# IamJasonBian/Splendor-RL-Gym

Measured on NVIDIA B200. Metric: expanded states/sec (gen+dedup+score+top-k), higher is better.
Workload: dtype u64 keys / f64 scores

## Files before the change

### splendor-rl-gym_b200/csrc/spl_kernels.cuh

```cuda
#pragma once
#include "spl_common.cuh"

namespace spl {

struct Counters {
    unsigned long long total_cands;
    unsigned long long n_new;
    unsigned long long n_emitted;
    unsigned long long sk_min, sk_max;
    long long goal_rank;
    unsigned int error;
    unsigned int ticket[4];
    unsigned long long key_or[2], key_and[2];
    unsigned long long n_buys;
    unsigned int n_runs, n_new_nodes;
    unsigned int n_cls[8];
    unsigned long long n_ties;
};

struct SelState {
    unsigned long long prefix;
    unsigned long long k_rem;
    unsigned long long c_gt;
    unsigned long long tie_count;
// ... 2 lines not shown
};

struct SmemTabs {
    uint64_t buy_lo[NCOL][8];
    uint64_t buy_hi[NCOL][8];
    uint32_t card[SPL_NUM_CARDS + 2];
};

__device__ __forceinline__ void load_tabs(SmemTabs &s, const DevTables *__restrict__ g) {
    const uint64_t *src = reinterpret_cast<const uint64_t *>(g);
    uint64_t *dst = reinterpret_cast<uint64_t *>(&s);
    for (int i = threadIdx.x; i < 2 * NCOL * 8; i += blockDim.x) dst[i] = src[i];
    for (int i = threadIdx.x; i < SPL_NUM_CARDS; i += blockDim.x) s.card[i] = g->card[i];
}

__device__ __forceinline__ void derive_parent(const SmemTabs &s, const uint32_t *__restrict__ takes_idx, uint64_t lo,
                                              uint64_t hi, uint64_t aux, uint64_t &bm_lo, uint64_t &bm_hi,
                                              uint32_t &nb, uint32_t &tk) {
    const uint32_t g = (uint32_t)(lo & GEM_MASK);
    bm_lo = ~lo;
    bm_hi = ~hi & HI_KEY_MASK;
#pragma unroll
    for (int c = 0; c < NCOL; ++c) {
        uint32_t v = ((g >> (3 * c)) & 7) + (uint32_t)((aux >> (24 + 5 * c)) & 31);
        v = v > 7 ? 7 : v;
        bm_lo &= s.buy_lo[c][v];
        bm_hi &= s.buy_hi[c][v];
    }
    nb = __popcll(bm_lo) + __popcll(bm_hi);
    tk = __ldg(takes_idx + g);
}

__device__ __forceinline__ int nth_set_bit64(uint64_t m, int n) {
    const uint32_t l = (uint32_t)m, h = (uint32_t)(m >> 32);
    const int c = __popc(l);
    return n < c ? nth_set_bit32(l, n) : 32 + nth_set_bit32(h, n - c);
}

__device__ __forceinline__ void make_child(const SmemTabs &s, const uint16_t *__restrict__ takes_edges, uint64_t lo,
                                           uint64_t hi, uint64_t aux, uint64_t bm_lo, uint64_t bm_hi, uint32_t nb,
                                           uint32_t tk, uint32_t ord, uint64_t &clo, uint64_t &chi, uint64_t &caux) {
    if (ord < nb) {
        const int c0 = __popcll(bm_lo);
        const int pos = (int)ord < c0 ? nth_set_bit64(bm_lo, ord) : 64 + nth_set_bit64(bm_hi, ord - c0);
        const uint32_t cd = s.card[pos - 15];
// ... 188 lines not shown
    cd = s.card[pos - 15];
    const uint32_t g = (uint32_t)(lo & GEM_MASK);
    uint32_t ng = 0;
    saved = 0;
#pragma unroll
    for (int c = 0; c < NCOL; ++c) {
        const int cost = (cd >> (3 * c)) & 7;
        const int b = (int)((aux >> (24 + 5 * c)) & 31);
        const int gc = (g >> (3 * c)) & 7;
        const int pay = max(cost - b, 0);
        saved += cost - pay;
        ng |= (uint32_t)max(gc - pay, 0) << (3 * c);
    }
    return ng;
}

constexpr int BUY_WIN = 4096;

struct ExpandSmem2 {
    SmemTabs tabs;
    uint64_t lo[TILE], hi[TILE], aux[TILE];
    uint32_t tk[TILE], nb[TILE], pref[TILE], prefb[TILE + 1];
    uint16_t units[TILE / 32][128];
    uint16_t blist[BUY_WIN];
    uint32_t warp_sums[TILE / 32 + 1];
};

template <int MODE, int IDENT>
__global__ void __launch_bounds__(TILE) expand_kernel(const Rec *__restrict__ front, int64_t n_par,
                                                      const DevTables *__restrict__ tabs,
// ... 58 lines not shown
                ++q;
            }
            m = bm_hi;
            while (m) {
                const int pos = 64 + __ffsll((long long)m) - 1;
                m &= m - 1;
                if (q >= w0 && q < w0 + BUY_WIN) S.blist[q - w0] = (uint16_t)(tid << 7 | pos);
                ++q;
            }
        }
        __syncthreads();
        const uint32_t nbw = min((uint32_t)BUY_WIN, total_buys - w0);
        for (uint32_t i = tid; i < nbw; i += TILE) {
            const uint32_t ent = S.blist[i], j = ent >> 7;
            const int pos = ent & 127;
            const uint64_t lo = S.lo[j], aux = S.aux[j];
            uint32_t saved, cd;
            const uint32_t ng = buy_gems(S.tabs, lo, aux, pos, saved, cd);
            uint64_t klo = (lo & ~GEM_MASK) | ng, khi = S.hi[j];
            if (pos < 64) klo |= 1ull << pos; else khi |= 1ull << (pos - 64);
            const uint32_t ord = w0 + i - S.prefb[j];
            const uint32_t tt = c0 + S.pref[j] + ord;
            if (MODE == MODE_PROBE) {
                cand_slot[tt] = probe_ident<IDENT>(table, cap, tag, klo, khi, ~(uint64_t)tt, n_new, &ctr->error);
            } else {
                const uint64_t caux = aux + saved + ((uint64_t)((cd >> 15) & 7) << 16) + (1ull << (24 + 5 * ((cd >> 18) & 7)));
                Rec r{klo, khi, caux, ((uint64_t)(rank_base + p0 + j) << 8) | ord};
                st_rec(cand_out + tt, r);
            }
        }
    }
    if (MODE == MODE_PROBE) {
#pragma unroll
        for (int d = 16; d; d >>= 1) n_new += __shfl_xor_sync(0xffffffffu, n_new, d);
        if (lane == 0 && n_new) atomicAdd(&ctr->n_new, (unsigned long long)n_new);
    }
}

template <int IDENT>
__global__ void __launch_bounds__(TILE) probe_list_kernel(const spl_key *__restrict__ keys, int64_t n,
                                                          uint64_t *__restrict__ table, uint64_t cap, uint64_t tag,
// ... 1025 lines not shown
```

### splendor-rl-gym_b200/csrc/spl_m2.cuh

```cuda
#pragma once
#include "spl_kernels.cuh"

namespace spl {

constexpr int GEM_STATES = 2898;
constexpr int NODE_BM_WORDS = 46;
constexpr int NODE_WORDS = 48;
constexpr uint64_t NODE_OCC = 1ull << 63;
constexpr int SMALL_ITEMS = 32;
constexpr int SMALL_W = 128;
constexpr int SM_TBL = 256;
constexpr int SM_STAGE = 48;
struct GroupArgs;
constexpr int NUM_CLS = 8;
constexpr int CLS_WARP = 6, CLS_CTA = 7;
constexpr int M2_WARPS = TILE / 32;
constexpr int BIG_DONE = 16;
constexpr int BIG_AT_BITS = 24;

__device__ __host__ __forceinline__ void mask_words(uint64_t lo, uint64_t hi, uint64_t &m0, uint64_t &m1) {
    m0 = (lo >> 15) | (hi << 49);
    m1 = (hi & HI_KEY_MASK) >> 15;
}
__device__ __host__ __forceinline__ uint64_t mask_hash(uint64_t m0, uint64_t m1) { return hash_key(m0, m1); }

__device__ __forceinline__ uint64_t node_find_or_create(uint64_t *__restrict__ nodes, uint64_t nn, uint64_t m0, uint64_t m1,
                                                        bool &fresh, unsigned int *error) {
    const uint64_t want1 = m1 | NODE_OCC;
    uint64_t i = __umul64hi(mask_hash(m0, m1), nn);
    fresh = false;
    for (int probes = 0; probes < MAX_PROBE; ++probes) {
        uint64_t *N = nodes + i * NODE_WORDS;
        uint64_t a, b;
// ... 74 lines not shown
    const uint32_t excl = block_excl_scan(nb, warp_sums, total);
    if (threadIdx.x < 32) {
        const uint64_t e = lookback_exclusive(status, tile, total, 0);
        if (threadIdx.x == 0) {
            s_base = e;
            if (total_tk) atomicAdd(&ctr->total_cands, (unsigned long long)total_tk);
            if ((int64_t)(tile + 1) * TILE >= np) ctr->n_buys = e + total;
        }
    }
    __syncthreads();
    if (p < np) boff[p] = (uint32_t)(s_base + excl);
}

struct BuySmem {
    SmemTabs tabs;
    uint64_t lo[TILE], hi[TILE], aux[TILE];
    uint32_t prefb[TILE + 1];
    uint16_t blist[BUY_WIN];
    uint32_t warp_sums[TILE / 32 + 1];
};
__global__ void __launch_bounds__(TILE) m2_buys_kernel(const Rec *__restrict__ front, int64_t np,
                                                       const DevTables *__restrict__ tabs,
                                                       const uint32_t *__restrict__ takes_idx,
                                                       const uint32_t *__restrict__ boff, int64_t rank_base,
                                                       Rec *__restrict__ brec, uint64_t *__restrict__ iv) {
    extern __shared__ __align__(16) unsigned char smem_raw[];
    BuySmem &S = *reinterpret_cast<BuySmem *>(smem_raw);
    const unsigned tid = threadIdx.x;
    load_tabs(S.tabs, tabs);
    __syncthreads();
    const int64_t p0 = (int64_t)blockIdx.x * TILE, p = p0 + tid;
    const uint32_t b0 = boff[p0];
    uint64_t bm_lo = 0, bm_hi = 0;
    uint32_t nb = 0, tk = 0;
    if (p < np) {
        Rec r;
        ld_rec(front + p, r);
        derive_parent(S.tabs, takes_idx, r.lo, r.hi, r.aux, bm_lo, bm_hi, nb, tk);
        S.lo[tid] = r.lo; S.hi[tid] = r.hi; S.aux[tid] = r.aux;
    }
    uint32_t total_buys;
    const uint32_t prefb = block_excl_scan(nb, S.warp_sums, total_buys);
    S.prefb[tid] = prefb;
    if (tid == 0) S.prefb[TILE] = total_buys;
    for (uint32_t w0 = 0; w0 < total_buys; w0 += BUY_WIN) {
        __syncthreads();
        {
            uint32_t q = prefb;
            uint64_t m = bm_lo;
            while (m) {
                const int pos = __ffsll((long long)m) - 1;
                m &= m - 1;
                if (q >= w0 && q < w0 + BUY_WIN) S.blist[q - w0] = (uint16_t)(tid << 7 | pos);
                ++q;
            }
            m = bm_hi;
            while (m) {
                const int pos = 64 + __ffsll((long long)m) - 1;
                m &= m - 1;
                if (q >= w0 && q < w0 + BUY_WIN) S.blist[q - w0] = (uint16_t)(tid << 7 | pos);
                ++q;
            }
        }
        __syncthreads();
        const uint32_t nbw = min((uint32_t)BUY_WIN, total_buys - w0);
        for (uint32_t i = tid; i < nbw; i += TILE) {
            const uint32_t ent = S.blist[i], j = ent >> 7;
            const int pos = ent & 127;
            const uint64_t lo = S.lo[j], aux = S.aux[j];
            uint32_t saved, cd;
            const uint32_t ng = buy_gems(S.tabs, lo, aux, pos, saved, cd);
            uint64_t klo = (lo & ~GEM_MASK) | ng, khi = S.hi[j];
            if (pos < 64) klo |= 1ull << pos; else khi |= 1ull << (pos - 64);
            const uint32_t ord = w0 + i - S.prefb[j];
            const uint64_t caux = aux + saved + ((uint64_t)((cd >> 15) & 7) << 16) + (1ull << (24 + 5 * ((cd >> 18) & 7)));
            const uint64_t g = (uint64_t)b0 + w0 + i;
            Rec r{klo, khi, caux, ((uint64_t)(rank_base + p0 + j) << 8) | ord};
            st_rec(brec + g, r);
            uint64_t m0, m1;
            mask_words(klo, khi, m0, m1);
            iv[np + g] = (mask_hash(m0, m1) & 0xFFFFFFFF00000000ull) | (uint64_t)(np + g);
        }
    }
}

__global__ void __launch_bounds__(TILE, 4) psort_scatter_kernel(const uint64_t *__restrict__ v_in, int64_t n, int shift,
                                                                const uint32_t *__restrict__ matrix_scanned, uint32_t ntiles,
                                                                uint64_t *__restrict__ v_out) {
    __shared__ uint32_t whist[TILE / 32][SORT_BINS];
    __shared__ uint32_t dbase[SORT_BINS], gbase[SORT_BINS];
    __shared__ uint32_t warp_sums[TILE / 32 + 1];
    __shared__ uint64_t stage[SORT_TILE];
    const unsigned lane = threadIdx.x & 31, w = threadIdx.x >> 5;
    for (int i = threadIdx.x; i < (TILE / 32) * SORT_BINS; i += TILE) (&whist[0][0])[i] = 0;
    __syncthreads();
    const int64_t tbase = (int64_t)blockIdx.x * SORT_TILE, wbase = tbase + (int64_t)w * (32 * SORT_ITEMS);
// ... 285 lines not shown
    uint64_t *nodes;
    uint64_t nn;
    Rec *out;
    uint64_t *out_sk;
    uint64_t out_base;
    uint32_t *cls_list[NUM_CLS];
    int h, noise_mode;
    ScoreLuts L;
    Counters *ctr;
};

__device__ __forceinline__ uint32_t item_id(const GroupArgs &A, uint32_t i) { return (uint32_t)A.iv[i]; }
__device__ __forceinline__ uint64_t parent_rank(const GroupArgs &A, uint32_t id) {
    return A.grank ? A.grank[id] : (uint64_t)(A.rank_base + id);
}

constexpr int M2_WARPS_ = TILE / 32;
struct WarpStage {
    uint64_t *st;
    uint32_t cnt;
    uint64_t kmin, kmax;
    __device__ __forceinline__ uint64_t &lo(uint32_t i) const { return st[i]; }
    __device__ __forceinline__ uint64_t &hi(uint32_t i) const { return st[1 * M2_WARPS_ * SM_STAGE + i]; }
    __device__ __forceinline__ uint64_t &aux(uint32_t i) const { return st[2 * M2_WARPS_ * SM_STAGE + i]; }
    __device__ __forceinline__ uint64_t &link(uint32_t i) const { return st[3 * M2_WARPS_ * SM_STAGE + i]; }
    __device__ __forceinline__ uint64_t &sk(uint32_t i) const { return st[4 * M2_WARPS_ * SM_STAGE + i]; }
};
__device__ __forceinline__ void stage_flush(const GroupArgs &A, WarpStage &W) {
    const unsigned lane = threadIdx.x & 31;
    __syncwarp();
// ... 93 lines not shown
    const bool act = q < (ptk & 0xff);
    const uint32_t g = act ? (uint32_t)__ldg(A.takes_edges + (ptk >> 8) + q) : 0u;
    bm_step(A, W, bm, act, true, g, (pgr << 8) | (pnb + q), (plo & ~GEM_MASK) | g, phi, paux);
}
__device__ __forceinline__ void take_steps(const GroupArgs &A, WarpStage &W, uint64_t *bm, uint64_t plo, uint64_t phi, uint64_t paux,
                                           uint64_t pgr, uint32_t ptk, uint32_t pnb) {
    const unsigned lane = threadIdx.x & 31;
    const uint32_t ntk = ptk & 0xff;
    for (uint32_t q0 = 0; q0 < ntk; q0 += 32) {
        const uint32_t q = q0 + lane;
        const bool act = q < ntk;
        const uint32_t g = act ? (uint32_t)__ldg(A.takes_edges + (ptk >> 8) + q) : 0u;
        bm_step(A, W, bm, act, false, g, (pgr << 8) | (pnb + q), (plo & ~GEM_MASK) | g, phi, paux);
    }
}
__device__ __forceinline__ void load_item(const GroupArgs &A, const SmemTabs &tabs, uint32_t i, Rec &it, bool &isP, uint32_t &nb,
                                          uint32_t &tk, uint64_t &grank, uint64_t &m0, uint64_t &m1) {
    const uint32_t id = item_id(A, i);
    isP = id < A.np;
    nb = tk = 0;
    grank = 0;
    if (isP) {
        ld_rec(A.front + id, it);
        uint64_t bl, bh;
        derive_parent(tabs, A.takes_idx, it.lo, it.hi, it.aux, bl, bh, nb, tk);
        grank = parent_rank(A, id);
    } else {
        ld_rec(A.brec + (id - A.np), it);
        grank = it.link >> 8;
    }
    mask_words(it.lo, it.hi, m0, m1);
}
__device__ __forceinline__ void warp_epilogue(const GroupArgs &A, WarpStage &W, uint32_t n_fresh) {
    const unsigned lane = threadIdx.x & 31;
    if (W.cnt) stage_flush(A, W);
    if (lane == 0 && n_fresh) atomicAdd(&A.ctr->n_new_nodes, n_fresh);
    if (A.out_sk) {
#pragma unroll
        for (int d = 16; d; d >>= 1) {
            W.kmin = min(W.kmin, __shfl_xor_sync(0xffffffffu, W.kmin, d));
            W.kmax = max(W.kmax, __shfl_xor_sync(0xffffffffu, W.kmax, d));
        }
        if (lane == 0 && W.kmin <= W.kmax) {
            atomicMin(&A.ctr->sk_min, (unsigned long long)W.kmin);
            atomicMax(&A.ctr->sk_max, (unsigned long long)W.kmax);
// ... 65 lines not shown
                        if (x > i) {
                            const uint64_t a = bs[i], b = bs[x];
                            if ((a > b) == ((i & k) == 0)) { bs[i] = b; bs[x] = a; }
                        }
                    }
                    __syncwarp();
                }
        }
        uint64_t (*done)[2] = S.done[w];
        int n_done = 0;
        uint32_t lead = s;
        while (lead != 0xFFFFFFFFu) {
            uint64_t M0 = 0, M1 = 0;
            if (lane == 0) {
                const uint32_t id = item_id(A, lead);
                const Rec *src = id < A.np ? A.front + id : A.brec + (id - A.np);
                mask_words(src->lo, src->hi, M0, M1);
            }
            M0 = __shfl_sync(0xffffffffu, M0, 0); M1 = __shfl_sync(0xffffffffu, M1, 0);
            uint64_t *N = node_open(A, M0, M1, bm, n_fresh);
            uint32_t next_lead = 0xFFFFFFFFu;
            Rec it{0, 0, 0, 0}, bt{0, 0, 0, 0};
            uint32_t nb = 0, tk = 0;
            uint64_t grank = 0, brank = 0;
            uint32_t bnext = pe, pnext = s;
            unsigned bmask = 0, pmask = 0;
            for (;;) {
                if (!pmask && pnext < pe) {
                    const bool valid = pnext + lane < pe;
                    bool p_;
                    uint64_t m0 = 0, m1 = 0;
                    if (valid) load_item(A, S.tabs, pnext + lane, it, p_, nb, tk, grank, m0, m1);
                    const bool ok = valid && m0 == M0 && m1 == M1;
                    bool other = valid && !ok;
#pragma unroll
                    for (int d = 0; d < MAX_SETS; ++d) other = other && !(d < n_done && done[d][0] == m0 && done[d][1] == m1);
                    const unsigned om = __ballot_sync(0xffffffffu, other);
                    if (om) next_lead = min(next_lead, pnext + (uint32_t)__ffs(om) - 1);
                    pmask = __ballot_sync(0xffffffffu, ok);
                    pnext += 32;
                    continue;
                }
                if (!bmask && bnext < e) {
                    const bool valid = bnext + lane < e;
                    uint64_t m0 = 0, m1 = 0;
                    if (valid) {
                        const uint32_t at = resort ? pe + (uint32_t)(bs[bnext - pe + lane] & 1023u) : bnext + lane;
                        ld_rec(A.brec + (item_id(A, at) - A.np), bt);
                        mask_words(bt.lo, bt.hi, m0, m1);
                        brank = bt.link >> 8;
                    }
                    const bool ok = valid && m0 == M0 && m1 == M1;
                    bool other = valid && !ok;
#pragma unroll
                    for (int d = 0; d < MAX_SETS; ++d) other = other && !(d < n_done && done[d][0] == m0 && done[d][1] == m1);
                    const unsigned om = __ballot_sync(0xffffffffu, other);
                    if (om) {
                        const uint32_t j = bnext - pe + (uint32_t)__ffs(om) - 1;
                        next_lead = min(next_lead, resort ? pe + (uint32_t)(bs[j] & 1023u) : pe + j);
                    }
                    bmask = __ballot_sync(0xffffffffu, ok);
                    bnext += 32;
                    continue;
// ... 35 lines not shown
        }
      }
    }
    warp_epilogue(A, W, n_fresh);
}

constexpr int TINY_ITEMS = 16;
#ifndef SPL_BIG_W
#define SPL_BIG_W 1024
#endif
constexpr uint32_t BIG_W = SPL_BIG_W;
template <bool UNORDERED>
__global__ void __launch_bounds__(TILE) m2_group_tiny_kernel(GroupArgs A, uint32_t n_runs) {
    __shared__ uint32_t warp_sums[TILE / 32 + 1];
    __shared__ uint64_t s_base;
    const unsigned lane = threadIdx.x & 31;
    const uint32_t r = blockIdx.x * TILE + threadIdx.x;
    int cls = -1;
    uint32_t s = 0, cnt = 0, winmask = 0;
    uint64_t *N = nullptr;
    uint32_t n_fresh = 0;
    uint64_t kmin = ~0ull, kmax = 0;
    if (r < n_runs) {
        s = A.run_start[r];
        cnt = A.run_start[r + 1] - s;
        const uint32_t id0 = item_id(A, s);
        const uint32_t wgt = A.run_wpre[r + 1] - A.run_wpre[r];
        if (cnt <= TINY_ITEMS && id0 >= A.np) cls = 0;
        else cls = wgt <= A.warp_max ? CLS_WARP : CLS_CTA;
        if (cls == 0) {
            uint64_t lo0, hi0, M0, M1;
            ld_cg_u64x2(reinterpret_cast<const uint64_t *>(A.brec + (id0 - A.np)), lo0, hi0);
            mask_words(lo0, hi0, M0, M1);
            uint32_t gp[TINY_ITEMS / 2];
#pragma unroll
            for (int q = 0; q < TINY_ITEMS / 2; ++q) gp[q] = 0;
            gp[0] = (uint32_t)(lo0 & GEM_MASK);
            bool same = true;
#pragma unroll
            for (int j = 1; j < TINY_ITEMS; ++j) {
                if (j < (int)cnt) {
                    uint64_t lo, hi, m0, m1;
                    ld_cg_u64x2(reinterpret_cast<const uint64_t *>(A.brec + (item_id(A, s + j) - A.np)), lo, hi);
                    mask_words(lo, hi, m0, m1);
                    same = same && m0 == M0 && m1 == M1;
                    gp[j >> 1] |= (uint32_t)(lo & GEM_MASK) << (16 * (j & 1));
                }
            }
            if (!same) {
                cls = CLS_WARP;
            } else {
                bool fresh;
                const uint64_t node = node_find_or_create(A.nodes, A.nn, M0, M1, fresh, &A.ctr->error);
                n_fresh = fresh;
                N = A.nodes + node * NODE_WORDS;
#pragma unroll
                for (int j = 0; j < TINY_ITEMS; ++j) {
                    if (j < (int)cnt) {
// ... 22 lines not shown
        if (m) {
            uint32_t base = 0;
            if (lane == (unsigned)(__ffs(m) - 1)) base = atomicAdd(&A.ctr->n_cls[k], (unsigned)__popc(m));
            base = __shfl_sync(0xffffffffu, base, __ffs(m) - 1);
            if (cls == k) A.cls_list[k][base + __popc(m & ((1u << lane) - 1))] = r;
        }
    }
    uint32_t tot;
    const uint32_t ex = block_excl_scan(__popc(winmask), warp_sums, tot);
    if (threadIdx.x == 0 && tot) s_base = A.out_base + atomicAdd(&A.ctr->n_emitted, (unsigned long long)tot);
    __syncthreads();
    uint64_t pos = s_base + ex;
    for (uint32_t m = winmask; m; m &= m - 1) {
        const int j = __ffs(m) - 1;
        Rec it;
        ld_rec(A.brec + (item_id(A, s + j) - A.np), it);
        st_rec(A.out + pos, it);
        const uint64_t k = flip_f64((uint64_t)__double_as_longlong(score_state(A.h, A.noise_mode, it.lo, it.hi & HI_KEY_MASK, it.aux, A.L)));
        A.out_sk[pos] = k;
        kmin = min(kmin, k); kmax = max(kmax, k);
        const uint32_t rk = __ldg(A.gemrank + (uint32_t)(it.lo & GEM_MASK));
        atomicOr(reinterpret_cast<unsigned long long *>(N + 2 + (rk >> 6)), 1ull << (rk & 63));
        ++pos;
    }
#pragma unroll
    for (int d = 16; d; d >>= 1) {
        n_fresh += __shfl_xor_sync(0xffffffffu, n_fresh, d);
        kmin = min(kmin, __shfl_xor_sync(0xffffffffu, kmin, d));
        kmax = max(kmax, __shfl_xor_sync(0xffffffffu, kmax, d));
    }
    if (lane == 0 && n_fresh) atomicAdd(&A.ctr->n_new_nodes, n_fresh);
// ... 1 lines not shown
        atomicMin(&A.ctr->sk_min, (unsigned long long)kmin);
        atomicMax(&A.ctr->sk_max, (unsigned long long)kmax);
    }
}

struct BigSmem {
    SmemTabs tabs;
    uint64_t tbl[GEM_STATES + 6];
    uint64_t bm[NODE_BM_WORDS];
    uint64_t done0[BIG_DONE], done1[BIG_DONE];
    uint32_t warp_sums[TILE / 32 + 1];
    uint32_t job, next, fresh, n_done;
    uint64_t node, base, m0, m1;
};

template <class F>
__device__ __forceinline__ void big_enumerate(const GroupArgs &A, BigSmem &S, uint32_t s, uint32_t e, uint64_t M0, uint64_t M1, F &&f) {
    for (uint32_t i = s + threadIdx.x; i < e; i += TILE) {
        const uint32_t id = item_id(A, i);
        Rec it;
        const bool isP = id < A.np;
        if (isP) ld_rec(A.front + id, it); else ld_rec(A.brec + (id - A.np), it);
        uint64_t m0, m1;
        mask_words(it.lo, it.hi, m0, m1);
        if (m0 != M0 || m1 != M1) {
            bool done = false;
            for (uint32_t d = 0; d < S.n_done; ++d) done |= (S.done0[d] == m0 && S.done1[d] == m1);
            if (!done) atomicMin(&S.next, i);
            continue;
        }
        if (!isP) {
            f((uint32_t)__ldg(A.gemrank + (uint32_t)(it.lo & GEM_MASK)), it.link, i - s);
        } else {
            uint64_t bl, bh;
            uint32_t nb, tk;
            derive_parent(S.tabs, A.takes_idx, it.lo, it.hi, it.aux, bl, bh, nb, tk);
            const uint64_t tb = (parent_rank(A, id) << 8) | nb;
            const uint32_t ntk = tk & 0xff;
            for (uint32_t q = 0; q < ntk; ++q) f((uint32_t)__ldg(A.gemrank + __ldg(A.takes_edges + (tk >> 8) + q)), tb + q, i - s);
        }
    }
}

__global__ void __launch_bounds__(TILE) m2_group_big_kernel(GroupArgs A) {
    extern __shared__ __align__(16) unsigned char smem_raw[];
    BigSmem &S = *reinterpret_cast<BigSmem *>(smem_raw);
    const unsigned tid = threadIdx.x, lane = tid & 31;
    load_tabs(S.tabs, A.tabs);
    const uint32_t n_big = A.ctr->n_cls[CLS_CTA];
    uint32_t n_fresh = 0;
    uint64_t kmin = ~0ull, kmax = 0;
    uint32_t ticket = 0;
    if (tid == 0) ticket = atomicAdd(&A.ctr->ticket[3], 1u);
    for (;;) {
        __syncthreads();
        if (tid == 0) {
            S.job = ticket;
            if (ticket < n_big) ticket = atomicAdd(&A.ctr->ticket[3], 1u);
        }
        __syncthreads();
        if (S.job >= n_big) break;
        const uint32_t r = A.cls_list[CLS_CTA][S.job];
        const uint32_t s = A.run_start[r], e = A.run_start[r + 1];
        if (tid == 0) { S.n_done = 0; S.next = s; }
        __syncthreads();
        while (S.next != 0xFFFFFFFFu) {
            const uint32_t lead = S.next;
            __syncthreads();
            if (tid == 0) {
                const uint32_t id = item_id(A, lead);
                const Rec *src = id < A.np ? A.front + id : A.brec + (id - A.np);
                mask_words(src->lo, src->hi, S.m0, S.m1);
                bool fresh;
                S.node = node_find_or_create(A.nodes, A.nn, S.m0, S.m1, fresh, &A.ctr->error);
                S.fresh = fresh;
                n_fresh += fresh;
                S.next = 0xFFFFFFFFu;
            }
            __syncthreads();
            const uint64_t M0 = S.m0, M1 = S.m1;
            uint64_t *N = A.nodes + S.node * NODE_WORDS;
            for (int i = tid; i < GEM_STATES; i += TILE) S.tbl[i] = ~0ull;
            if (tid < NODE_BM_WORDS) S.bm[tid] = S.fresh ? 0ull : N[2 + tid];
            __syncthreads();
            big_enumerate(A, S, s, e, M0, M1, [&](uint32_t rk, uint64_t t, uint32_t at) {
                if (!((S.bm[rk >> 6] >> (rk & 63)) & 1))
                    atomicMin(reinterpret_cast<unsigned long long *>(&S.tbl[rk]), (unsigned long long)((t << BIG_AT_BITS) | at));
            });
            __syncthreads();
            uint32_t mywins = 0;
            for (uint32_t rk = tid; rk < GEM_STATES; rk += TILE) mywins += S.tbl[rk] != ~0ull;
            uint32_t tot;
            const uint32_t ex = block_excl_scan(mywins, S.warp_sums, tot);
            if (tid == 0) S.base = A.out_base + atomicAdd(&A.ctr->n_emitted, (unsigned long long)tot);
            __syncthreads();
            uint64_t pos = S.base + ex;
            for (uint32_t rk = tid; rk < GEM_STATES; rk += TILE) {
                const uint64_t v = S.tbl[rk];
                if (v == ~0ull) continue;
                const uint32_t id = item_id(A, s + (uint32_t)(v & ((1u << BIG_AT_BITS) - 1)));
                Rec o;
                if (id < A.np) {
                    ld_rec(A.front + id, o);
                    o.lo = (o.lo & ~GEM_MASK) | __ldg(A.rankgems + rk);
                } else {
                    ld_rec(A.brec + (id - A.np), o);
                }
                o.link = v >> BIG_AT_BITS;
                st_rec(A.out + pos, o);
                if (A.out_sk) {
                    const uint64_t k = flip_f64((uint64_t)__double_as_longlong(score_state(A.h, A.noise_mode, o.lo, o.hi & HI_KEY_MASK, o.aux, A.L)));
                    A.out_sk[pos] = k;
                    kmin = min(kmin, k); kmax = max(kmax, k);
                }
                ++pos;
                atomicOr(reinterpret_cast<unsigned *>(S.bm) + (rk >> 5), 1u << (rk & 31));
            }
            __syncthreads();
            if (tid < NODE_BM_WORDS) N[2 + tid] = S.bm[tid];
            if (tid == 0) {
                if (S.n_done < BIG_DONE) { S.done0[S.n_done] = M0; S.done1[S.n_done] = M1; ++S.n_done; }
// ... 21 lines not shown
```

### splendor-rl-gym_b200/csrc/splendor_b200.cu

```cuda
#include "../../include/splendor_b200.h"

#include <stdarg.h>
#include <stdio.h>
#include <string.h>

#include <algorithm>
#include <string>
#include <vector>

#include "spl_kernels.cuh"
#include "spl_m2.cuh"
#include "spl_shard.cuh"
#include "spl_realistic.cuh"
#include "spl_tables.cuh"

using namespace spl;

static std::string g_create_error;

struct DevBuf {
    void *p = nullptr;
    size_t cap = 0;
    ~DevBuf() { release(); }
    void release() {
        if (p) cudaFree(p);
        p = nullptr;
        cap = 0;
    }
    cudaError_t ensure(size_t bytes, size_t keep, cudaStream_t st) {
        if (bytes <= cap) return cudaSuccess;
        size_t ncap = std::max(bytes, cap + cap / 2);
// ... 86 lines not shown
    int grow(spl_ctx *c, uint64_t need, cudaStream_t st);
};

struct spl_ctx {
    int device = 0;
    std::string err;
    VisitTable key{KEY_TABLE_DESC}, nodes{NODE_TABLE_DESC}, rtab{REALISTIC_TABLE_DESC};
    uint64_t occupied = 0;
    uint32_t epoch = 0;
    uint64_t chunk_parents = 0;
    bool chunk_user = false;
    uint64_t link_budget = 0;
    uint64_t spilled_bytes = 0;
    uint16_t *d_gemrank = nullptr;
    uint16_t *d_rankgems = nullptr;
    DevBuf brec, ntk8, boff2, run_start, run_wpre, cls_list;
    DevTables *d_tabs = nullptr;
    uint32_t *d_takes_idx = nullptr;
    uint16_t *d_takes_edges = nullptr;
    double *d_lut = nullptr;
    ScoreLuts luts{};
    Counters *d_ctr = nullptr, *h_ctr = nullptr;
    SelState *d_sel = nullptr, *h_sel = nullptr;
    uint32_t *d_hist = nullptr;
    ScoreDict *d_dict = nullptr, *d_dict2 = nullptr;
    unsigned long long *d_dest = nullptr;
    int dict_skip = 0;
    int identity = IDENT_KEY;
    DevBuf status[3];
    DevBuf off, cand_slot, tmp_rec, tmp_rec2, sk, y[2], idx[2], kl[2], kh[2], matrix, matrix2, os_hist, os_status;
    DevBuf pool_front, pool_uniq, pool_grank;
// ... 109 lines not shown
    do {                                                                                                      \
        cudaError_t e2_ = (call);                                                                             \
        if (e2_ != cudaSuccess) {                                                                             \
            cudaGetLastError();                                                                               \
            int r_ = fail(nullptr, e2_ == cudaErrorMemoryAllocation ? SPL_E_NOMEM : SPL_E_CUDA, "%s: %s", #call, \
                          cudaGetErrorString(e2_));                                                           \
            delete c;                                                                                         \
            return r_;                                                                                        \
        }                                                                                                     \
    } while (0)
    CKC(cudaSetDevice(c->device));
    size_t free_b = 0, total_b = 0;
    CKC(cudaMemGetInfo(&free_b, &total_b));
    c->key.max_bytes = c->rtab.max_bytes = cfg->max_table_bytes ? cfg->max_table_bytes : (uint64_t)(free_b * 0.6);
    c->chunk_user = cfg->chunk_parents != 0;
    c->chunk_parents = cfg->chunk_parents ? std::min<uint64_t>(cfg->chunk_parents, 16ull << 20) : (4ull << 20);
    c->chunk_parents = std::max<uint64_t>(c->chunk_parents, TILE);
    const HostTables &T = host_tables();
    CKC(cudaMalloc(&c->d_tabs, sizeof(DevTables)));
    CKC(cudaMemcpy(c->d_tabs, &T.dev, sizeof(DevTables), cudaMemcpyHostToDevice));
    CKC(cudaMalloc(&c->d_takes_idx, T.takes_idx.size() * 4));
    CKC(cudaMemcpy(c->d_takes_idx, T.takes_idx.data(), T.takes_idx.size() * 4, cudaMemcpyHostToDevice));
    CKC(cudaMalloc(&c->d_takes_edges, T.takes_edges.size() * 2));
    CKC(cudaMemcpy(c->d_takes_edges, T.takes_edges.data(), T.takes_edges.size() * 2, cudaMemcpyHostToDevice));
    const size_t n_lut = T.lut_pts.size() + T.lut_saved.size() + T.lut_small.size();
    CKC(cudaMalloc(&c->d_lut, n_lut * 8));
    CKC(cudaMemcpy(c->d_lut, T.lut_pts.data(), T.lut_pts.size() * 8, cudaMemcpyHostToDevice));
    CKC(cudaMemcpy(c->d_lut + T.lut_pts.size(), T.lut_saved.data(), T.lut_saved.size() * 8, cudaMemcpyHostToDevice));
    CKC(cudaMemcpy(c->d_lut + T.lut_pts.size() + T.lut_saved.size(), T.lut_small.data(), T.lut_small.size() * 8,
                   cudaMemcpyHostToDevice));
    c->luts.pts = c->d_lut;
// ... 10 lines not shown
    }
    CKC(cudaMalloc(&c->d_ctr, sizeof(Counters)));
    CKC(cudaMallocHost(&c->h_ctr, sizeof(Counters)));
    CKC(cudaMalloc(&c->d_sel, sizeof(SelState)));
    CKC(cudaMallocHost(&c->h_sel, sizeof(SelState)));
    CKC(cudaMalloc(&c->d_hist, SEL_BINS * 4));
    CKC(cudaMemset(c->d_hist, 0, SEL_BINS * 4));
    CKC(cudaMalloc(&c->d_dict, sizeof(ScoreDict)));
    for (auto &ev : c->ev) CKC(cudaEventCreate(&ev));
    CKC(cudaFuncSetAttribute(expand_kernel<MODE_PROBE, IDENT_KEY>, cudaFuncAttributeMaxDynamicSharedMemorySize, (int)sizeof(ExpandSmem2)));
    CKC(cudaFuncSetAttribute(expand_kernel<MODE_PROBE, IDENT_PYHASH>, cudaFuncAttributeMaxDynamicSharedMemorySize, (int)sizeof(ExpandSmem2)));
    CKC(cudaFuncSetAttribute(expand_kernel<MODE_LIST, IDENT_KEY>, cudaFuncAttributeMaxDynamicSharedMemorySize, (int)sizeof(ExpandSmem2)));
    CKC(cudaFuncSetAttribute(m2_buys_kernel, cudaFuncAttributeMaxDynamicSharedMemorySize, (int)sizeof(BuySmem)));
    CKC(cudaFuncSetAttribute(m2_group_warp_kernel<false>, cudaFuncAttributeMaxDynamicSharedMemorySize, (int)offsetof(WarpSmem, bsort)));
    CKC(cudaFuncSetAttribute(m2_group_warp_kernel<true>, cudaFuncAttributeMaxDynamicSharedMemorySize, (int)sizeof(WarpSmem)));
    CKC(cudaFuncSetAttribute(m2_group_big_kernel, cudaFuncAttributeMaxDynamicSharedMemorySize, (int)sizeof(BigSmem)));
    CKC(cudaFuncSetAttribute(os_scatter_kernel<false>, cudaFuncAttributeMaxDynamicSharedMemorySize, (int)offsetof(OsSmem, stage_p)));
    CKC(cudaFuncSetAttribute(os_scatter_kernel<true>, cudaFuncAttributeMaxDynamicSharedMemorySize, (int)sizeof(OsSmem)));
    CKC(cudaFuncSetAttribute(gs_buys_route_kernel, cudaFuncAttributeMaxDynamicSharedMemorySize, (int)sizeof(RouteSmem)));
    CKC(cudaMalloc(&c->d_dict2, sizeof(ScoreDict)));
    CKC(cudaMalloc(&c->d_dest, 3 * MAX_RANKS * 8));
    {
        c->nodes.max_bytes = cfg->max_node_bytes ? cfg->max_node_bytes : (uint64_t)(free_b * 0.5);
        uint64_t nn = cfg->node_slots ? cfg->node_slots : (1ull << 12);
        nn = std::max<uint64_t>(std::min<uint64_t>(nn, c->nodes.max_bytes / (NODE_WORDS * 8)), 64);
        CKC(c->nodes.alloc(nn, 0));
    }
    c->rslots_hint = cfg->table_slots;
    uint64_t slots = cfg->table_slots ? cfg->table_slots : (1ull << 22);
    slots = std::min<uint64_t>(slots, c->key.max_bytes / 64 * BUCKET_SLOTS);
    slots = std::max<uint64_t>(slots, 1024);
// ... 1019 lines not shown
    A.warp_max = R.unordered ? std::min<uint32_t>(BIG_W, BSORT_MAX) : BIG_W;
    A.tabs = c->d_tabs; A.takes_idx = c->d_takes_idx; A.takes_edges = c->d_takes_edges; A.gemrank = c->d_gemrank; A.rankgems = c->d_rankgems;
    A.nodes = c->nodes.as<uint64_t>(); A.nn = c->nodes.units; A.out = R.out->as<Rec>(); A.out_sk = c->sk.as<uint64_t>(); A.out_base = (uint64_t)R.out_base;
    for (int k = 0; k < NUM_CLS; ++k) A.cls_list[k] = nullptr;
    A.cls_list[CLS_WARP] = c->cls_list.as<uint32_t>();
    A.cls_list[CLS_CTA] = c->cls_list.as<uint32_t>() + n_runs;
    A.h = R.heuristic; A.noise_mode = R.noise; A.L = c->luts; A.ctr = c->d_ctr;
    CK(c, cudaEventRecord(c->ev[3], st));
    if (R.unordered) m2_group_tiny_kernel<true><<<nblk((int64_t)n_runs), TILE, 0, st>>>(A, (uint32_t)n_runs);
    else m2_group_tiny_kernel<false><<<nblk((int64_t)n_runs), TILE, 0, st>>>(A, (uint32_t)n_runs);
    CK(c, cudaEventRecord(c->ev[4], st));
    CKS(c, reset_ticket(c, 2, st));
    if (R.unordered) m2_group_warp_kernel<true><<<148 * SPL_WARP_CTAS, TILE, sizeof(WarpSmem), st>>>(A);
    else m2_group_warp_kernel<false><<<148 * SPL_WARP_CTAS, TILE, offsetof(WarpSmem, bsort), st>>>(A);
    CK(c, cudaEventRecord(c->ev[5], st));
    m2_group_big_kernel<<<148 * 5, TILE, sizeof(BigSmem), st>>>(A);
    c->launches += 3;
    CK(c, cudaGetLastError());
    CK(c, cudaEventRecord(c->ev[6], st));
    CKS(c, read_ctr(c, st));
    const Counters &h = *c->h_ctr;
    cudaEventElapsedTime(&t->sort, c->ev[1], c->ev[2]);
    cudaEventElapsedTime(&t->prep, c->ev[2], c->ev[3]);
    cudaEventElapsedTime(&t->thread, c->ev[3], c->ev[4]);
    cudaEventElapsedTime(&t->warp, c->ev[4], c->ev[5]);
    cudaEventElapsedTime(&t->cta, c->ev[5], c->ev[6]);
    if (getenv("SPL_DEBUG"))
        fprintf(stderr, "[grouped] L%d np=%lld items=%lld runs=%llu cls=%u/%u/%u new_nodes=%u winners=%llu | sort+runs %.2f prep %.2f thread %.2f warp %.2f cta %.2f ms | nodes %llu/%llu\n",
                R.level, (long long)R.np, (long long)R.n_items, (unsigned long long)n_runs,
                (unsigned)(n_runs - h.n_cls[CLS_WARP] - h.n_cls[CLS_CTA]), h.n_cls[CLS_WARP], h.n_cls[CLS_CTA], h.n_new_nodes,
                (unsigned long long)h.n_emitted, t->sort, t->prep, t->thread, t->warp, t->cta, (unsigned long long)c->nodes.occ,
// ... 1 lines not shown
    c->nodes.occ += h.n_new_nodes;
    if (h.error == 3)
        return fail(c, SPL_E_CUDA, "level %d: more than %d card sets share one 30-bit sort key in a run of the warp kernel (or more than %d in one of the CTA kernel)",
                    R.level, MAX_SETS + 1, BIG_DONE + 1);
    if (h.error)
        return fail(c, SPL_E_TABLE_FULL, "card-set table full during level %d (device error %u; %llu slots, max_node_bytes=%llu)", R.level,
                    h.error, (unsigned long long)c->nodes.units, (unsigned long long)c->nodes.max_bytes);
    c->occupied += h.n_emitted;
    *n_new_out = (int64_t)h.n_emitted;
    return SPL_OK;
}

static int grouped_expand(spl_solver *s, int64_t n, LevelExpand *x, float ms[6], cudaStream_t st) {
    spl_ctx *c = s->c;
    const Rec *front = s->front.as<Rec>();
    const int64_t chunk = c->chunk_user ? (int64_t)c->chunk_parents : (16ll << 20);
    int64_t n_uniq = 0, n_slots = 0, generated = 0;
    uint64_t sk_min = ~0ull, sk_max = 0;
    for (int64_t p0 = 0; p0 < n; p0 += chunk) {
        const int64_t np = std::min<int64_t>(chunk, n - p0);
        const unsigned nt = nblk(np);
        CKS(c, zero_ctr(c, st));
        CK(c, cudaEventRecord(c->ev[0], st));
        CK(c, c->boff2.ensure((size_t)np * 4 + 4, 0, st));
        CK(c, c->ntk8.ensure((size_t)np + 8, 0, st));
        CK(c, c->y[0].ensure((size_t)np * 8 + 8, 0, st));
        CKS(c, prep_status(c, 0, nt, st));
        m2_count_kernel<<<nt, TILE, 0, st>>>(front + p0, np, c->d_tabs, c->d_takes_idx, c->boff2.as<uint32_t>(),
                                              c->y[0].as<uint64_t>(), c->ntk8.as<uint8_t>(), c->status[0].as<uint64_t>(), c->d_ctr, 0);
        ++c->launches;
        CK(c, cudaGetLastError());
        CKS(c, read_ctr(c, st));
        const uint64_t n_takes = c->h_ctr->total_cands, n_buys = c->h_ctr->n_buys, total = n_takes + n_buys;
        generated += (int64_t)total;
        if (total == 0) continue;
        const int64_t n_items = np + (int64_t)n_buys;
        if (total >= 0xFFFFFFFFull || (uint64_t)n_items >= 0xFFFFFFFFull)
            return fail(c, SPL_E_INVALID, "round produced %llu candidates (>= 2^32): lower spl_config.chunk_parents", (unsigned long long)total);
        CK(c, c->y[0].ensure((size_t)n_items * 8 + 8, (size_t)np * 8, st));
        CK(c, c->y[1].ensure((size_t)n_items * 8 + 8, 0, st));
        CK(c, c->brec.ensure((size_t)n_buys * 32 + 32, 0, st));
        if (n_buys) {
            m2_buys_kernel<<<nt, TILE, sizeof(BuySmem), st>>>(front + p0, np, c->d_tabs, c->d_takes_idx, c->boff2.as<uint32_t>(), p0,
                                                               c->brec.as<Rec>(), c->y[0].as<uint64_t>());
            ++c->launches;
            CK(c, cudaGetLastError());
        }
        GroupRound R;
        R.front = front + p0; R.brec = c->brec.as<Rec>(); R.np = np; R.n_items = n_items; R.n_cands = total; R.rank_base = p0;
        R.out = &s->uniq; R.out_base = n_slots; R.heuristic = s->heuristic; R.noise = s->noise; R.level = s->level;
        int64_t n_new = 0;
        RoundTimes t;
        CKS(c, group_round(c, R, &n_new, &t, st));
        if (n_new) { sk_min = std::min<uint64_t>(sk_min, c->h_ctr->sk_min); sk_max = std::max<uint64_t>(sk_max, c->h_ctr->sk_max); }
        n_uniq += n_new;
        n_slots += n_new;
        float t_count;
        cudaEventElapsedTime(&t_count, c->ev[0], c->ev[1]);
        ms[0] += t_count;
        ms[2] += t.sort;
        ms[1] += t.thread + t.warp + t.cta;
        ms[5] += t.warp;
    }
    *x = LevelExpand{n_uniq, n_slots, generated, sk_min, sk_max};
// ... 1172 lines not shown
```

Baseline: 658.5 million.

## Recompute buy children from parent on demand instead of materializing buy records

```diff
diff --git a/splendor-rl-gym_b200/csrc/spl_kernels.cuh b/splendor-rl-gym_b200/csrc/spl_kernels.cuh
--- a/splendor-rl-gym_b200/csrc/spl_kernels.cuh
+++ b/splendor-rl-gym_b200/csrc/spl_kernels.cuh
@@ -40,9 +40,8 @@
     for (int i = threadIdx.x; i < SPL_NUM_CARDS; i += blockDim.x) s.card[i] = g->card[i];
 }
 
-__device__ __forceinline__ void derive_parent(const SmemTabs &s, const uint32_t *__restrict__ takes_idx, uint64_t lo,
-                                              uint64_t hi, uint64_t aux, uint64_t &bm_lo, uint64_t &bm_hi,
-                                              uint32_t &nb, uint32_t &tk) {
+__device__ __forceinline__ void buy_mask(const SmemTabs &s, uint64_t lo, uint64_t hi, uint64_t aux, uint64_t &bm_lo,
+                                         uint64_t &bm_hi) {
     const uint32_t g = (uint32_t)(lo & GEM_MASK);
     bm_lo = ~lo;
     bm_hi = ~hi & HI_KEY_MASK;
@@ -53,8 +52,13 @@
         bm_lo &= s.buy_lo[c][v];
         bm_hi &= s.buy_hi[c][v];
     }
+}
+__device__ __forceinline__ void derive_parent(const SmemTabs &s, const uint32_t *__restrict__ takes_idx, uint64_t lo,
+                                              uint64_t hi, uint64_t aux, uint64_t &bm_lo, uint64_t &bm_hi,
+                                              uint32_t &nb, uint32_t &tk) {
+    buy_mask(s, lo, hi, aux, bm_lo, bm_hi);
     nb = __popcll(bm_lo) + __popcll(bm_hi);
-    tk = __ldg(takes_idx + g);
+    tk = __ldg(takes_idx + (uint32_t)(lo & GEM_MASK));
 }
 
 __device__ __forceinline__ int nth_set_bit64(uint64_t m, int n) {
@@ -273,6 +277,21 @@
     }
     return ng;
 }
+__device__ __forceinline__ void set_key_bit(uint64_t &lo, uint64_t &hi, int pos) {
+    if (pos < 64) lo |= 1ull << pos; else hi |= 1ull << (pos - 64);
+}
+__device__ __forceinline__ void buy_child(const SmemTabs &s, uint64_t lo, uint64_t hi, uint64_t aux, int pos, uint64_t &clo,
+                                          uint64_t &chi, uint64_t &caux) {
+    uint32_t saved, cd;
+    const uint32_t ng = buy_gems(s, lo, aux, pos, saved, cd);
+    clo = (lo & ~GEM_MASK) | ng;
+    chi = hi;
+    set_key_bit(clo, chi, pos);
+    caux = aux + saved + ((uint64_t)((cd >> 15) & 7) << 16) + (1ull << (24 + 5 * ((cd >> 18) & 7)));
+}
+__device__ __forceinline__ uint32_t buy_ordinal(uint64_t bm_lo, uint64_t bm_hi, int pos) {
+    return pos < 64 ? __popcll(bm_lo & ((1ull << pos) - 1)) : __popcll(bm_lo) + __popcll(bm_hi & ((1ull << (pos - 64)) - 1));
+}
 
 constexpr int BUY_WIN = 4096;
 
@@ -361,17 +380,13 @@
         for (uint32_t i = tid; i < nbw; i += TILE) {
             const uint32_t ent = S.blist[i], j = ent >> 7;
             const int pos = ent & 127;
-            const uint64_t lo = S.lo[j], aux = S.aux[j];
-            uint32_t saved, cd;
-            const uint32_t ng = buy_gems(S.tabs, lo, aux, pos, saved, cd);
-            uint64_t klo = (lo & ~GEM_MASK) | ng, khi = S.hi[j];
-            if (pos < 64) klo |= 1ull << pos; else khi |= 1ull << (pos - 64);
+            uint64_t klo, khi, caux;
+            buy_child(S.tabs, S.lo[j], S.hi[j], S.aux[j], pos, klo, khi, caux);
             const uint32_t ord = w0 + i - S.prefb[j];
             const uint32_t tt = c0 + S.pref[j] + ord;
             if (MODE == MODE_PROBE) {
                 cand_slot[tt] = probe_ident<IDENT>(table, cap, tag, klo, khi, ~(uint64_t)tt, n_new, &ctr->error);
             } else {
-                const uint64_t caux = aux + saved + ((uint64_t)((cd >> 15) & 7) << 16) + (1ull << (24 + 5 * ((cd >> 18) & 7)));
                 Rec r{klo, khi, caux, ((uint64_t)(rank_base + p0 + j) << 8) | ord};
                 st_rec(cand_out + tt, r);
             }
diff --git a/splendor-rl-gym_b200/csrc/spl_m2.cuh b/splendor-rl-gym_b200/csrc/spl_m2.cuh
--- a/splendor-rl-gym_b200/csrc/spl_m2.cuh
+++ b/splendor-rl-gym_b200/csrc/spl_m2.cuh
@@ -17,6 +17,9 @@
 constexpr int M2_WARPS = TILE / 32;
 constexpr int BIG_DONE = 16;
 constexpr int BIG_AT_BITS = 24;
+constexpr int ITEM_PARENT_BITS = 24;
+constexpr uint32_t ITEM_BUY = 1u << 31;
+__device__ __forceinline__ uint32_t buy_item_id(uint32_t p, int pos) { return ITEM_BUY | p << 7 | (uint32_t)pos; }
 
 __device__ __host__ __forceinline__ void mask_words(uint64_t lo, uint64_t hi, uint64_t &m0, uint64_t &m1) {
     m0 = (lo >> 15) | (hi << 49);
@@ -121,7 +124,7 @@
 
 struct BuySmem {
     SmemTabs tabs;
-    uint64_t lo[TILE], hi[TILE], aux[TILE];
+    uint64_t lo[TILE], hi[TILE];
     uint32_t prefb[TILE + 1];
     uint16_t blist[BUY_WIN];
     uint32_t warp_sums[TILE / 32 + 1];
@@ -129,8 +132,7 @@
 __global__ void __launch_bounds__(TILE) m2_buys_kernel(const Rec *__restrict__ front, int64_t np,
                                                        const DevTables *__restrict__ tabs,
                                                        const uint32_t *__restrict__ takes_idx,
-                                                       const uint32_t *__restrict__ boff, int64_t rank_base,
-                                                       Rec *__restrict__ brec, uint64_t *__restrict__ iv) {
+                                                       const uint32_t *__restrict__ boff, uint64_t *__restrict__ iv) {
     extern __shared__ __align__(16) unsigned char smem_raw[];
     BuySmem &S = *reinterpret_cast<BuySmem *>(smem_raw);
     const unsigned tid = threadIdx.x;
@@ -144,7 +146,7 @@
         Rec r;
         ld_rec(front + p, r);
         derive_parent(S.tabs, takes_idx, r.lo, r.hi, r.aux, bm_lo, bm_hi, nb, tk);
-        S.lo[tid] = r.lo; S.hi[tid] = r.hi; S.aux[tid] = r.aux;
+        S.lo[tid] = r.lo; S.hi[tid] = r.hi;
     }
     uint32_t total_buys;
     const uint32_t prefb = block_excl_scan(nb, S.warp_sums, total_buys);
@@ -174,19 +176,11 @@
         for (uint32_t i = tid; i < nbw; i += TILE) {
             const uint32_t ent = S.blist[i], j = ent >> 7;
             const int pos = ent & 127;
-            const uint64_t lo = S.lo[j], aux = S.aux[j];
-            uint32_t saved, cd;
-            const uint32_t ng = buy_gems(S.tabs, lo, aux, pos, saved, cd);
-            uint64_t klo = (lo & ~GEM_MASK) | ng, khi = S.hi[j];
-            if (pos < 64) klo |= 1ull << pos; else khi |= 1ull << (pos - 64);
-            const uint32_t ord = w0 + i - S.prefb[j];
-            const uint64_t caux = aux + saved + ((uint64_t)((cd >> 15) & 7) << 16) + (1ull << (24 + 5 * ((cd >> 18) & 7)));
+            uint64_t klo = S.lo[j], khi = S.hi[j], m0, m1;
+            set_key_bit(klo, khi, pos);
+            mask_words(klo, khi, m0, m1);
             const uint64_t g = (uint64_t)b0 + w0 + i;
-            Rec r{klo, khi, caux, ((uint64_t)(rank_base + p0 + j) << 8) | ord};
-            st_rec(brec + g, r);
-            uint64_t m0, m1;
-            mask_words(klo, khi, m0, m1);
-            iv[np + g] = (mask_hash(m0, m1) & 0xFFFFFFFF00000000ull) | (uint64_t)(np + g);
+            iv[np + g] = (mask_hash(m0, m1) & 0xFFFFFFFF00000000ull) | buy_item_id((uint32_t)(p0 + j), pos);
         }
     }
 }
@@ -502,6 +496,32 @@
 __device__ __forceinline__ uint64_t parent_rank(const GroupArgs &A, uint32_t id) {
     return A.grank ? A.grank[id] : (uint64_t)(A.rank_base + id);
 }
+template <bool UNORDERED>
+__device__ __forceinline__ void load_buy(const GroupArgs &A, const SmemTabs &tabs, uint32_t id, Rec &b) {
+    if (UNORDERED) {
+        ld_rec(A.brec + (id - A.np), b);
+        return;
+    }
+    const uint32_t p = (id >> 7) & ((1u << ITEM_PARENT_BITS) - 1);
+    const int pos = id & 127;
+    Rec par;
+    ld_rec(A.front + p, par);
+    buy_child(tabs, par.lo, par.hi, par.aux, pos, b.lo, b.hi, b.aux);
+    uint64_t bl, bh;
+    buy_mask(tabs, par.lo, par.hi, par.aux, bl, bh);
+    b.link = (uint64_t)(A.rank_base + p) << 8 | buy_ordinal(bl, bh, pos);
+}
+template <bool UNORDERED>
+__device__ __forceinline__ void load_buy_key(const GroupArgs &A, const SmemTabs &tabs, uint32_t id, uint64_t &lo, uint64_t &hi) {
+    if (UNORDERED) {
+        ld_cg_u64x2(reinterpret_cast<const uint64_t *>(A.brec + (id - A.np)), lo, hi);
+        return;
+    }
+    Rec b;
+    load_buy<false>(A, tabs, id, b);
+    lo = b.lo;
+    hi = b.hi;
+}
 
 constexpr int M2_WARPS_ = TILE / 32;
 struct WarpStage {
@@ -625,21 +645,13 @@
         bm_step(A, W, bm, act, false, g, (pgr << 8) | (pnb + q), (plo & ~GEM_MASK) | g, phi, paux);
     }
 }
-__device__ __forceinline__ void load_item(const GroupArgs &A, const SmemTabs &tabs, uint32_t i, Rec &it, bool &isP, uint32_t &nb,
-                                          uint32_t &tk, uint64_t &grank, uint64_t &m0, uint64_t &m1) {
+__device__ __forceinline__ void load_parent_item(const GroupArgs &A, const SmemTabs &tabs, uint32_t i, Rec &it, uint32_t &nb,
+                                                 uint32_t &tk, uint64_t &grank, uint64_t &m0, uint64_t &m1) {
     const uint32_t id = item_id(A, i);
-    isP = id < A.np;
-    nb = tk = 0;
-    grank = 0;
-    if (isP) {
-        ld_rec(A.front + id, it);
-        uint64_t bl, bh;
-        derive_parent(tabs, A.takes_idx, it.lo, it.hi, it.aux, bl, bh, nb, tk);
-        grank = parent_rank(A, id);
-    } else {
-        ld_rec(A.brec + (id - A.np), it);
-        grank = it.link >> 8;
-    }
+    ld_rec(A.front + id, it);
+    uint64_t bl, bh;
+    derive_parent(tabs, A.takes_idx, it.lo, it.hi, it.aux, bl, bh, nb, tk);
+    grank = parent_rank(A, id);
     mask_words(it.lo, it.hi, m0, m1);
 }
 __device__ __forceinline__ void warp_epilogue(const GroupArgs &A, WarpStage &W, uint32_t n_fresh) {
@@ -735,8 +747,9 @@
             uint64_t M0 = 0, M1 = 0;
             if (lane == 0) {
                 const uint32_t id = item_id(A, lead);
-                const Rec *src = id < A.np ? A.front + id : A.brec + (id - A.np);
-                mask_words(src->lo, src->hi, M0, M1);
+                Rec src;
+                if (id < A.np) ld_rec(A.front + id, src); else load_buy<UNORDERED>(A, S.tabs, id, src);
+                mask_words(src.lo, src.hi, M0, M1);
             }
             M0 = __shfl_sync(0xffffffffu, M0, 0); M1 = __shfl_sync(0xffffffffu, M1, 0);
             uint64_t *N = node_open(A, M0, M1, bm, n_fresh);
@@ -749,9 +762,8 @@
             for (;;) {
                 if (!pmask && pnext < pe) {
                     const bool valid = pnext + lane < pe;
-                    bool p_;
                     uint64_t m0 = 0, m1 = 0;
-                    if (valid) load_item(A, S.tabs, pnext + lane, it, p_, nb, tk, grank, m0, m1);
+                    if (valid) load_parent_item(A, S.tabs, pnext + lane, it, nb, tk, grank, m0, m1);
                     const bool ok = valid && m0 == M0 && m1 == M1;
                     bool other = valid && !ok;
 #pragma unroll
@@ -767,7 +779,7 @@
                     uint64_t m0 = 0, m1 = 0;
                     if (valid) {
                         const uint32_t at = resort ? pe + (uint32_t)(bs[bnext - pe + lane] & 1023u) : bnext + lane;
-                        ld_rec(A.brec + (item_id(A, at) - A.np), bt);
+                        load_buy<UNORDERED>(A, S.tabs, item_id(A, at), bt);
                         mask_words(bt.lo, bt.hi, m0, m1);
                         brank = bt.link >> 8;
                     }
@@ -833,6 +845,11 @@
 __global__ void __launch_bounds__(TILE) m2_group_tiny_kernel(GroupArgs A, uint32_t n_runs) {
     __shared__ uint32_t warp_sums[TILE / 32 + 1];
     __shared__ uint64_t s_base;
+    __shared__ SmemTabs tabs;
+    if (!UNORDERED) {
+        load_tabs(tabs, A.tabs);
+        __syncthreads();
+    }
     const unsigned lane = threadIdx.x & 31;
     const uint32_t r = blockIdx.x * TILE + threadIdx.x;
     int cls = -1;
@@ -849,7 +866,7 @@
         else cls = wgt <= A.warp_max ? CLS_WARP : CLS_CTA;
         if (cls == 0) {
             uint64_t lo0, hi0, M0, M1;
-            ld_cg_u64x2(reinterpret_cast<const uint64_t *>(A.brec + (id0 - A.np)), lo0, hi0);
+            load_buy_key<UNORDERED>(A, tabs, id0, lo0, hi0);
             mask_words(lo0, hi0, M0, M1);
             uint32_t gp[TINY_ITEMS / 2];
 #pragma unroll
@@ -860,7 +877,7 @@
             for (int j = 1; j < TINY_ITEMS; ++j) {
                 if (j < (int)cnt) {
                     uint64_t lo, hi, m0, m1;
-                    ld_cg_u64x2(reinterpret_cast<const uint64_t *>(A.brec + (item_id(A, s + j) - A.np)), lo, hi);
+                    load_buy_key<UNORDERED>(A, tabs, item_id(A, s + j), lo, hi);
                     mask_words(lo, hi, m0, m1);
                     same = same && m0 == M0 && m1 == M1;
                     gp[j >> 1] |= (uint32_t)(lo & GEM_MASK) << (16 * (j & 1));
@@ -913,7 +930,7 @@
     for (uint32_t m = winmask; m; m &= m - 1) {
         const int j = __ffs(m) - 1;
         Rec it;
-        ld_rec(A.brec + (item_id(A, s + j) - A.np), it);
+        load_buy<UNORDERED>(A, tabs, item_id(A, s + j), it);
         st_rec(A.out + pos, it);
         const uint64_t k = flip_f64((uint64_t)__double_as_longlong(score_state(A.h, A.noise_mode, it.lo, it.hi & HI_KEY_MASK, it.aux, A.L)));
         A.out_sk[pos] = k;
@@ -945,13 +962,13 @@
     uint64_t node, base, m0, m1;
 };
 
-template <class F>
+template <bool UNORDERED, class F>
 __device__ __forceinline__ void big_enumerate(const GroupArgs &A, BigSmem &S, uint32_t s, uint32_t e, uint64_t M0, uint64_t M1, F &&f) {
     for (uint32_t i = s + threadIdx.x; i < e; i += TILE) {
         const uint32_t id = item_id(A, i);
         Rec it;
         const bool isP = id < A.np;
-        if (isP) ld_rec(A.front + id, it); else ld_rec(A.brec + (id - A.np), it);
+        if (isP) ld_rec(A.front + id, it); else load_buy<UNORDERED>(A, S.tabs, id, it);
         uint64_t m0, m1;
         mask_words(it.lo, it.hi, m0, m1);
         if (m0 != M0 || m1 != M1) {
@@ -973,6 +990,7 @@
     }
 }
 
+template <bool UNORDERED>
 __global__ void __launch_bounds__(TILE) m2_group_big_kernel(GroupArgs A) {
     extern __shared__ __align__(16) unsigned char smem_raw[];
     BigSmem &S = *reinterpret_cast<BigSmem *>(smem_raw);
@@ -1000,8 +1018,9 @@
             __syncthreads();
             if (tid == 0) {
                 const uint32_t id = item_id(A, lead);
-                const Rec *src = id < A.np ? A.front + id : A.brec + (id - A.np);
-                mask_words(src->lo, src->hi, S.m0, S.m1);
+                Rec src;
+                if (id < A.np) ld_rec(A.front + id, src); else load_buy<UNORDERED>(A, S.tabs, id, src);
+                mask_words(src.lo, src.hi, S.m0, S.m1);
                 bool fresh;
                 S.node = node_find_or_create(A.nodes, A.nn, S.m0, S.m1, fresh, &A.ctr->error);
                 S.fresh = fresh;
@@ -1014,7 +1033,7 @@
             for (int i = tid; i < GEM_STATES; i += TILE) S.tbl[i] = ~0ull;
             if (tid < NODE_BM_WORDS) S.bm[tid] = S.fresh ? 0ull : N[2 + tid];
             __syncthreads();
-            big_enumerate(A, S, s, e, M0, M1, [&](uint32_t rk, uint64_t t, uint32_t at) {
+            big_enumerate<UNORDERED>(A, S, s, e, M0, M1, [&](uint32_t rk, uint64_t t, uint32_t at) {
                 if (!((S.bm[rk >> 6] >> (rk & 63)) & 1))
                     atomicMin(reinterpret_cast<unsigned long long *>(&S.tbl[rk]), (unsigned long long)((t << BIG_AT_BITS) | at));
             });
@@ -1035,7 +1054,7 @@
                     ld_rec(A.front + id, o);
                     o.lo = (o.lo & ~GEM_MASK) | __ldg(A.rankgems + rk);
                 } else {
-                    ld_rec(A.brec + (id - A.np), o);
+                    load_buy<UNORDERED>(A, S.tabs, id, o);
                 }
                 o.link = v >> BIG_AT_BITS;
                 st_rec(A.out + pos, o);
diff --git a/splendor-rl-gym_b200/csrc/splendor_b200.cu b/splendor-rl-gym_b200/csrc/splendor_b200.cu
--- a/splendor-rl-gym_b200/csrc/splendor_b200.cu
+++ b/splendor-rl-gym_b200/csrc/splendor_b200.cu
@@ -15,6 +15,9 @@
 #include "spl_tables.cuh"
 
 using namespace spl;
+
+constexpr uint64_t MAX_CHUNK_PARENTS = 16ull << 20;
+static_assert(MAX_CHUNK_PARENTS <= (1ull << ITEM_PARENT_BITS), "a round's parent index must fit the item of its buys");
 
 static std::string g_create_error;
 
@@ -131,7 +134,7 @@
     uint64_t spilled_bytes = 0;
     uint16_t *d_gemrank = nullptr;
     uint16_t *d_rankgems = nullptr;
-    DevBuf brec, ntk8, boff2, run_start, run_wpre, cls_list;
+    DevBuf ntk8, boff2, run_start, run_wpre, cls_list;
     DevTables *d_tabs = nullptr;
     uint32_t *d_takes_idx = nullptr;
     uint16_t *d_takes_edges = nullptr;
@@ -271,7 +274,7 @@
     CKC(cudaMemGetInfo(&free_b, &total_b));
     c->key.max_bytes = c->rtab.max_bytes = cfg->max_table_bytes ? cfg->max_table_bytes : (uint64_t)(free_b * 0.6);
     c->chunk_user = cfg->chunk_parents != 0;
-    c->chunk_parents = cfg->chunk_parents ? std::min<uint64_t>(cfg->chunk_parents, 16ull << 20) : (4ull << 20);
+    c->chunk_parents = cfg->chunk_parents ? std::min<uint64_t>(cfg->chunk_parents, MAX_CHUNK_PARENTS) : (4ull << 20);
     c->chunk_parents = std::max<uint64_t>(c->chunk_parents, TILE);
     const HostTables &T = host_tables();
     CKC(cudaMalloc(&c->d_tabs, sizeof(DevTables)));
@@ -312,7 +315,8 @@
     CKC(cudaFuncSetAttribute(m2_buys_kernel, cudaFuncAttributeMaxDynamicSharedMemorySize, (int)sizeof(BuySmem)));
     CKC(cudaFuncSetAttribute(m2_group_warp_kernel<false>, cudaFuncAttributeMaxDynamicSharedMemorySize, (int)offsetof(WarpSmem, bsort)));
     CKC(cudaFuncSetAttribute(m2_group_warp_kernel<true>, cudaFuncAttributeMaxDynamicSharedMemorySize, (int)sizeof(WarpSmem)));
-    CKC(cudaFuncSetAttribute(m2_group_big_kernel, cudaFuncAttributeMaxDynamicSharedMemorySize, (int)sizeof(BigSmem)));
+    CKC(cudaFuncSetAttribute(m2_group_big_kernel<false>, cudaFuncAttributeMaxDynamicSharedMemorySize, (int)sizeof(BigSmem)));
+    CKC(cudaFuncSetAttribute(m2_group_big_kernel<true>, cudaFuncAttributeMaxDynamicSharedMemorySize, (int)sizeof(BigSmem)));
     CKC(cudaFuncSetAttribute(os_scatter_kernel<false>, cudaFuncAttributeMaxDynamicSharedMemorySize, (int)offsetof(OsSmem, stage_p)));
     CKC(cudaFuncSetAttribute(os_scatter_kernel<true>, cudaFuncAttributeMaxDynamicSharedMemorySize, (int)sizeof(OsSmem)));
     CKC(cudaFuncSetAttribute(gs_buys_route_kernel, cudaFuncAttributeMaxDynamicSharedMemorySize, (int)sizeof(RouteSmem)));
@@ -1362,7 +1366,8 @@
     if (R.unordered) m2_group_warp_kernel<true><<<148 * SPL_WARP_CTAS, TILE, sizeof(WarpSmem), st>>>(A);
     else m2_group_warp_kernel<false><<<148 * SPL_WARP_CTAS, TILE, offsetof(WarpSmem, bsort), st>>>(A);
     CK(c, cudaEventRecord(c->ev[5], st));
-    m2_group_big_kernel<<<148 * 5, TILE, sizeof(BigSmem), st>>>(A);
+    if (R.unordered) m2_group_big_kernel<true><<<148 * 5, TILE, sizeof(BigSmem), st>>>(A);
+    else m2_group_big_kernel<false><<<148 * 5, TILE, sizeof(BigSmem), st>>>(A);
     c->launches += 3;
     CK(c, cudaGetLastError());
     CK(c, cudaEventRecord(c->ev[6], st));
@@ -1394,7 +1399,7 @@
 static int grouped_expand(spl_solver *s, int64_t n, LevelExpand *x, float ms[6], cudaStream_t st) {
     spl_ctx *c = s->c;
     const Rec *front = s->front.as<Rec>();
-    const int64_t chunk = c->chunk_user ? (int64_t)c->chunk_parents : (16ll << 20);
+    const int64_t chunk = c->chunk_user ? (int64_t)c->chunk_parents : (int64_t)MAX_CHUNK_PARENTS;
     int64_t n_uniq = 0, n_slots = 0, generated = 0;
     uint64_t sk_min = ~0ull, sk_max = 0;
     for (int64_t p0 = 0; p0 < n; p0 += chunk) {
@@ -1419,15 +1424,14 @@
             return fail(c, SPL_E_INVALID, "round produced %llu candidates (>= 2^32): lower spl_config.chunk_parents", (unsigned long long)total);
         CK(c, c->y[0].ensure((size_t)n_items * 8 + 8, (size_t)np * 8, st));
         CK(c, c->y[1].ensure((size_t)n_items * 8 + 8, 0, st));
-        CK(c, c->brec.ensure((size_t)n_buys * 32 + 32, 0, st));
         if (n_buys) {
-            m2_buys_kernel<<<nt, TILE, sizeof(BuySmem), st>>>(front + p0, np, c->d_tabs, c->d_takes_idx, c->boff2.as<uint32_t>(), p0,
-                                                               c->brec.as<Rec>(), c->y[0].as<uint64_t>());
+            m2_buys_kernel<<<nt, TILE, sizeof(BuySmem), st>>>(front + p0, np, c->d_tabs, c->d_takes_idx, c->boff2.as<uint32_t>(),
+                                                               c->y[0].as<uint64_t>());
             ++c->launches;
             CK(c, cudaGetLastError());
         }
         GroupRound R;
-        R.front = front + p0; R.brec = c->brec.as<Rec>(); R.np = np; R.n_items = n_items; R.n_cands = total; R.rank_base = p0;
+        R.front = front + p0; R.np = np; R.n_items = n_items; R.n_cands = total; R.rank_base = p0;
         R.out = &s->uniq; R.out_base = n_slots; R.heuristic = s->heuristic; R.noise = s->noise; R.level = s->level;
         int64_t n_new = 0;
         RoundTimes t;
```

Result: faster. 684.4 million (median of 6 runs) (+3.9%).
